# alexj94/future_urban_scene_generation

Measured on NVIDIA B200. Metric: vehicle crops/s novel-view completion (warp+VUNet), higher is better.
Workload: dtype bf16

## Files before the change

future_urban_scene_generation_b200/_lib.py:

```python
import ctypes as C
import os

_HERE = os.path.dirname(os.path.abspath(__file__))
LIB_PATH = os.path.join(_HERE, "libfusg.so")

POLY_COORD_MAX = 1 << 20
ERRORS = {-1: "FUSG_ERR_ARG", -2: "FUSG_ERR_UNSUPPORTED", -3: "FUSG_ERR_CUDA", -4: "FUSG_ERR_WORKSPACE"}


class FusgError(RuntimeError):
    pass


def _load():
    if not os.path.exists(LIB_PATH):
        raise FusgError(
            f"{LIB_PATH} not found: build it with `python -c 'import __graft_entry__ as g; g.build()'` "
            "(nvcc, sm_100a).  There is no CPU fallback for this path.")
    lib = C.CDLL(LIB_PATH)
    vp, sz, i = C.c_void_p, C.c_size_t, C.c_int
    sigs = {
        "fusg_version": ([], i),
        "fusg_last_error": ([], C.c_char_p),
        "fusg_kernel_launches": ([], i),
        "fusg_warp_workspace_bytes": ([i], sz),
        "fusg_warp_workspace_bytes_hw": ([i, i, i], sz),
        "fusg_warp_fused": ([vp] * 11 + [vp, sz, i, i, i, vp], i),
        "fusg_warp_fused_traj": ([vp] * 12 + [vp, sz, i, i, i, vp], i),
        "fusg_warp_fused_idx": ([vp, vp, i] + [vp] * 11 + [vp, sz, i, i, i, vp], i),
        "fusg_warp_window_workspace_bytes": ([i, i, i], sz),
        "fusg_warp_fused_window": ([vp, vp, i] + [vp] * 9 + [i] + [vp] * 4 + [vp, sz, i, i, i, vp], i),
        "fusg_step_keypoints": ([vp] * 10 + [i, i, i, vp], i),
        "fusg_visibility": ([vp] * 6 + [i, i, i, vp], i),
        "fusg_get_planes": ([vp] * 3 + [i, i, i, vp], i),
        "fusg_find_homography": ([vp, vp, i, vp, vp, i, vp], i),
        "fusg_warp_perspective": ([vp] * 3 + [i, i, i, vp], i),
        "fusg_conv2d": ([vp, vp], i),
        "fusg_conv2d_select": ([vp], i),
        "fusg_conv2d_last_plan": ([vp], None),
        "fusg_conv2d_set_sm_reserve": ([i], i),
        "fusg_sizeof_conv_desc": ([], sz),
        "fusg_fold_weightnorm": ([vp, vp, vp, i, i, i, i, i, i, vp], i),
        "fusg_fold_weightnorm_paired": ([vp, vp, vp, vp, vp, i, i, i, i, i, i, vp], i),
        "fusg_nchw_to_nhwc": ([vp, vp, i, i, i, i, i, i, i, vp], i),
        "fusg_nhwc_to_nchw": ([vp, vp, i, i, i, i, i, i, vp], i),
        "fusg_to_image": ([vp, vp, i, i, i, vp], i),
        "fusg_to_image_lab": ([vp, vp, vp, vp, i, i, i, vp], i),
        "fusg_elu": ([vp, vp, sz, i, vp], i),
        "fusg_nchw_to_nhwc_reflect": ([vp, vp, i, i, i, i, i, i, i, vp], i),
        "fusg_norm_stats": ([vp, vp, i, i, i, i, i, vp], i),
        "fusg_norm_finalize": ([vp, vp, vp, vp, i, i, i, i, i, C.c_float, vp], i),
        "fusg_norm_apply": ([vp, vp, vp, i, vp, i, i, i, i, i, i, i, i, vp], i),
        "fusg_resize_u8": ([vp] * 6 + [i, i, vp], i),
        "fusg_paste_workspace_bytes": ([i, i, i], sz),
# ... 26 lines not shown
    return _lib


def check(rc, what):
    if rc != 0:
        msg = lib().fusg_last_error().decode() if rc == -3 else ""
        raise FusgError(f"{what} failed: {ERRORS.get(rc, rc)} {msg}")


def conv_last_plan():
    buf = (C.c_int32 * 8)()
    lib().fusg_conv2d_last_plan(buf)
    return dict(zip(("msub", "pair", "halo", "ksplit", "stages", "group", "w_resident", "fast_epi"), list(buf)))


def kernel_launches():
    return lib().fusg_kernel_launches()


def require_cuda():
    import torch
    if not torch.cuda.is_available():
        raise FusgError("no CUDA device: the B200 path has no CPU fallback")
    return torch


def ptr(t):
    if t is None:
        return None
    assert t.is_cuda and t.is_contiguous(), "expected a contiguous CUDA tensor"
# ... 6 lines not shown
```

future_urban_scene_generation_b200/csrc/conv.cu:

```cuda
#include <cuda.h>
#include <cuda_bf16.h>
#include <cuda_fp16.h>
#include <type_traits>
#include <cuda_runtime.h>
#include <cstdint>
#include <cstdio>
#include <cstring>
#include "../../include/fusg.h"
#include "fusg_common.h"

namespace fusg {

__device__ __forceinline__ float elu1(float x) {
    float e;
    asm("ex2.approx.ftz.f32 %0, %1;" : "=f"(e) : "f"(x * 1.4426950408889634f));
    return x > 0.f ? x : e - 1.f;
}

template <typename T> __device__ __forceinline__ float to_f(T v);
template <> __device__ __forceinline__ float to_f<float>(float v) { return v; }
template <> __device__ __forceinline__ float to_f<__nv_bfloat16>(__nv_bfloat16 v) { return __bfloat162float(v); }
template <> __device__ __forceinline__ float to_f<__half>(__half v) { return __half2float(v); }
template <typename T> __device__ __forceinline__ T from_f(float v);
template <> __device__ __forceinline__ float from_f<float>(float v) { return v; }
// ... 163 lines not shown
    }
    if (active) epilogue16<T>(d, d.bias, Ho, Wo, b, y, x, n0, acc);
}

__device__ __forceinline__ uint32_t s_addr(const void *p) { return (uint32_t)__cvta_generic_to_shared(p); }

__device__ __forceinline__ void mbar_init(uint64_t *bar, uint32_t count) {
    asm volatile("mbarrier.init.shared::cta.b64 [%0], %1;" ::"r"(s_addr(bar)), "r"(count));
}
__device__ __forceinline__ void mbar_arrive_expect_tx(uint64_t *bar, uint32_t bytes) {
    asm volatile("mbarrier.arrive.expect_tx.shared::cta.b64 _, [%0], %1;" ::"r"(s_addr(bar)), "r"(bytes) : "memory");
}
__device__ __forceinline__ void mbar_arrive(uint64_t *bar) {
    asm volatile("mbarrier.arrive.shared::cta.b64 _, [%0];" ::"r"(s_addr(bar)) : "memory");
}
constexpr unsigned TC_WAIT_COUNTER_OFF = 312;
__device__ __forceinline__ void mbar_wait(uint64_t *bar, uint32_t parity) {
    uint32_t done = 0;
    while (!done) {
        asm volatile(
            "{\n\t.reg .pred p;\n\t"
            "mbarrier.try_wait.parity.shared::cta.b64 p, [%1], %2, %3;\n\t"
            "selp.u32 %0, 1, 0, p;\n\t}"
            : "=r"(done)
            : "r"(s_addr(bar)), "r"(parity), "r"(0x989680u)
            : "memory");
        if (!done) fusg_wait_failed((s_addr(bar) & ~1023u) + TC_WAIT_COUNTER_OFF);
    }
}
__device__ __forceinline__ void tma_load_4d(void *dst, const CUtensorMap *tm, uint64_t *bar, int c0, int c1, int c2, int c3) {
    asm volatile(
// ... 237 lines not shown
            v.x = __uint_as_float(acc[c]) + s_bias[c];
            v.y = __uint_as_float(acc[cq + c]) + s_bias[cq + c];
            *reinterpret_cast<float2 *>(p + c * plane) = v;
        }
    }
}

constexpr int TC_EPI_WARPS = 8;
constexpr int TC_THREADS = 64 + 32 * TC_EPI_WARPS;
constexpr int TC_STAGING_BYTES = 32768;
constexpr int TC_STAGE_BYTES = TC_STAGING_BYTES / TC_EPI_WARPS;
constexpr int TC_BLOCK_M = 128;
constexpr int TC_HALO_ROWS_MAX = TC_BLOCK_M + 6;
constexpr int TC_HALO_BYTES = ((TC_HALO_ROWS_MAX * 128 + 1023) / 1024) * 1024;
constexpr int TC_MAX_STAGES = 16;
static_assert(TC_WAIT_COUNTER_OFF == (2 * TC_MAX_STAGES + 5) * 8 + 16, "the wait guard's start-time slot must be tmem_slot[4]");

struct alignas(64) ConvTcParams {
    CUtensorMap tmA0, tmA1, tmW;
    fusg_conv_desc d;
    int Ho, Wo;
    int Wt, Ht, Bt;
    int wt_shift, ht_shift;
    int txs, tys;
    int msub;
    int tiles_x, tiles_y, tiles_b;
    int n_tiles, block_n;
    int kc;
    int chunks0, chunks1;
    int num_kblocks;
    int stages;
    int a_bytes, b_bytes;
    int group;
    int w_resident;
    int halo;
    int hks;
    uint32_t halo_skip;
    int pair;
    int epi_smem;
    unsigned long long w_prefetch_bytes;
    int ksplit;
    int kb_local;
    int tmem_cols;
    int fast_epi;
    FastEpi fe;
};

struct TcSmem { size_t b, bias, stage, total; };
__host__ __device__ __forceinline__ TcSmem tc_smem(const ConvTcParams &p) {
    const size_t pipe_a = p.halo ? (size_t)p.stages * 2 * TC_HALO_BYTES : (size_t)p.stages * p.group * p.a_bytes;
    const size_t pipe_b = p.w_resident ? (size_t)p.num_kblocks * p.b_bytes
                                       : (p.halo ? (size_t)p.stages * p.hks * p.b_bytes : (size_t)p.stages * p.group * p.b_bytes);
    TcSmem s;
    s.b = 1024 + pipe_a;
    s.bias = s.b + ((pipe_b + 15) & ~(size_t)15);
    s.stage = s.bias + (size_t)p.d.cout_pad * 4;
    s.total = 1024  + s.b + pipe_b + 16  + (size_t)p.d.cout_pad * 4 + (size_t)p.epi_smem;
    return s;
}

template <int KSTEPS, int MSUB>
__device__ __forceinline__ void mma_role(const ConvTcParams &p, uint8_t *sA, uint8_t *sB, uint64_t *full_bar, uint64_t *empty_bar,
                                         uint64_t *tfull_bar, uint64_t *tempty_bar, uint64_t *w_bar, uint32_t tmem_base, int total_tiles) {
    const uint32_t block_n = (uint32_t)p.block_n;
    const uint32_t idesc = (1u << 4) | (p.fe.f16 ? 0u : ((1u << 7) | (1u << 10))) | ((block_n >> 3) << 17) | ((uint32_t)(TC_BLOCK_M >> 4) << 24);
    const uint32_t kc = KSTEPS * 16;
    const uint64_t desc_hi = ((uint64_t)1 << 16) | ((uint64_t)((kc * 2u * 8u) >> 4) << 32) | ((uint64_t)1 << 46) | ((uint64_t)(KSTEPS == 4 ? 2u : 4u) << 61);
    const uint32_t sub16 = (TC_BLOCK_M * kc * 2u) >> 4;
    const int group = p.group, stages = p.stages, groups = p.kb_local / p.group;
    const uint32_t a_kb16 = (uint32_t)p.a_bytes >> 4, b_kb16 = (uint32_t)p.b_bytes >> 4;
    const uint32_t a_stage16 = a_kb16 * group, b_stage16 = b_kb16 * group;
    const bool resident = p.w_resident != 0;
    const uint32_t sA16 = (s_addr(sA) & 0x3FFFF) >> 4, sB16 = (s_addr(sB) & 0x3FFFF) >> 4;
    const uint32_t acc_cols = (uint32_t)MSUB * block_n;
    int stage = 0;
    uint32_t phase = 0;
// ... 17 lines not shown
#pragma unroll
                        for (int ks = 0; ks < KSTEPS; ++ks) {
                            umma_bf16(d_tmem + (uint32_t)sub * block_n, a_desc + (uint64_t)(sub * sub16 + ks * 2), b_desc + (uint64_t)(ks * 2), idesc,
                                      ks == 0 ? first : 1u);
                        }
                    }
                    a16 += a_kb16;
                    b16 += b_kb16;
                }
                umma_commit(&empty_bar[stage]);
                if (grp == groups - 1) umma_commit(&tfull_bar[acc]);
            }
            __syncwarp();
            if (++stage == stages) { stage = 0; phase ^= 1; }
        }
        acc ^= 1;
        if (acc == 0) acc_phase ^= 1;
    }
}

template <bool PAIR, int KS>
__device__ __forceinline__ void mma_role_halo(const ConvTcParams &p, uint8_t *sA, uint8_t *sB, uint64_t *full_bar, uint64_t *empty_bar,
                                              uint64_t *tfull_bar, uint64_t *tempty_bar, uint64_t *w_bar, uint32_t tmem_base, int total_tiles) {
    const uint32_t block_n = (uint32_t)p.block_n;
    constexpr bool pair = PAIR;
    if (pair && cluster_ctarank() != 0) return;
    const uint32_t idesc = (1u << 4) | (p.fe.f16 ? 0u : ((1u << 7) | (1u << 10))) | ((block_n >> 3) << 17) | ((uint32_t)((pair ? 2 * TC_BLOCK_M : TC_BLOCK_M) >> 4) << 24);
    const uint64_t desc_hi = ((uint64_t)1 << 16) | ((uint64_t)(1024u >> 4) << 32) | ((uint64_t)1 << 46) | ((uint64_t)2u << 61);
    const int stages = p.stages, cpt = p.chunks0 + p.chunks1, nst = KS * cpt;
    const uint32_t skip = p.halo_skip;
    int st_first = 0, st_last = nst - 1;
    while ((skip >> st_first) & 1u) ++st_first;
    while ((skip >> st_last) & 1u) --st_last;
    const uint32_t b_kb16 = (uint32_t)p.b_bytes >> 4;
    const uint32_t a_stage16 = (2u * TC_HALO_BYTES) >> 4, b_stage16 = (uint32_t)KS * b_kb16;
    const bool resident = p.w_resident != 0;
// ... 36 lines not shown
                } else {
#pragma unroll 1
                    for (int kx = 0; kx < KS; ++kx) issue_tap(kx);
                }
                if constexpr (PAIR) {
                    umma_commit_2cta(&empty_bar[stage]);
                    if (st == st_last) umma_commit_2cta(&tfull_bar[acc]);
                } else {
                    umma_commit(&empty_bar[stage]);
                    if (st == st_last) umma_commit(&tfull_bar[acc]);
                }
            }
            __syncwarp();
            if (++stage == stages) { stage = 0; phase ^= 1; }
        }
        acc ^= 1;
        if (acc == 0) acc_phase ^= 1;
    }
}

template <bool PAIR>
__global__ void __launch_bounds__(TC_THREADS, 1) k_conv_tc(const __grid_constant__ ConvTcParams p) {
    extern __shared__ __align__(1024) uint8_t smem_raw[];
    uint8_t *smem = reinterpret_cast<uint8_t *>((reinterpret_cast<uintptr_t>(smem_raw) + 1023) & ~(uintptr_t)1023);
    const TcSmem lay = tc_smem(p);
    uint64_t *bars = reinterpret_cast<uint64_t *>(smem);
    uint8_t *sA = smem + 1024;
    uint8_t *sB = smem + lay.b;
    uint64_t *full_bar = bars, *empty_bar = bars + TC_MAX_STAGES, *tfull_bar = bars + 2 * TC_MAX_STAGES, *tempty_bar = tfull_bar + 2;
    uint64_t *w_bar = tempty_bar + 2;
    uint32_t *tmem_slot = reinterpret_cast<uint32_t *>(w_bar + 1);
    float *s_bias = reinterpret_cast<float *>(smem + lay.bias);
    uint8_t *s_stage = reinterpret_cast<uint8_t *>(s_bias + p.d.cout_pad);
    float *s_recv = reinterpret_cast<float *>(s_stage);

    const int warp = threadIdx.x >> 5, lane = threadIdx.x & 31;
    const fusg_conv_desc &d = p.d;

    if (warp == 0 && lane == 0) {
        tma_prefetch_desc(&p.tmA0);
        if (d.in1) tma_prefetch_desc(&p.tmA1);
        tma_prefetch_desc(&p.tmW);
        for (int s = 0; s < p.stages; ++s) { mbar_init(&full_bar[s], 1); mbar_init(&empty_bar[s], 1); }
        for (int a = 0; a < 2; ++a) { mbar_init(&tfull_bar[a], 1); mbar_init(&tempty_bar[a], PAIR ? 2 * TC_EPI_WARPS : TC_EPI_WARPS); }
        mbar_init(w_bar, 1);
        fusg_wait_guard_start(tmem_slot + 4);
        asm volatile("fence.mbarrier_init.release.cluster;" ::: "memory");
    }
    if (warp == 1) {
        if constexpr (PAIR) tmem_alloc2(tmem_slot, (uint32_t)p.tmem_cols);
        else tmem_alloc(tmem_slot, (uint32_t)p.tmem_cols);
    }
    for (int i = threadIdx.x; i < p.d.cout_pad; i += TC_THREADS) s_bias[i] = p.d.bias[i];
    tc_fence_before();
    __syncthreads();
    if constexpr (PAIR) cluster_sync_all();
    tc_fence_after();
    const uint32_t tmem_base = *tmem_slot;
    if (p.w_prefetch_bytes && threadIdx.x == 32) {
        const unsigned long long total = p.w_prefetch_bytes, per = ((total / gridDim.x) + 15ull) & ~15ull;
        unsigned long long lo = per * blockIdx.x, hi = lo + per < total ? lo + per : total;
        const char *wb = reinterpret_cast<const char *>(d.weight);
        for (; lo < hi; lo += 32768ull) {
            const unsigned n = (unsigned)(hi - lo < 32768ull ? hi - lo : 32768ull) & ~15u;
            if (n) asm volatile("cp.async.bulk.prefetch.L2.global [%0], %1;" ::"l"(wb + lo), "r"(n) : "memory");
        }
    }
    asm volatile("griddepcontrol.wait;" ::: "memory");
    asm volatile("griddepcontrol.launch_dependents;" ::: "memory");
    if (p.ksplit > 1) asm volatile("barrier.cluster.arrive.relaxed.aligned;" ::: "memory");

    const int m_tiles = p.tiles_x * p.tiles_y * p.tiles_b;
    const int total_tiles = m_tiles * p.n_tiles;
    const int pad = d.pad_mode ? d.pad - d.border : d.ksize >> 1;
    const int cpt = p.chunks0 + p.chunks1;
    int split_tile = -1;

    if (warp == 0) {
        {
            const int groups = p.kb_local / p.group;
            const int kb0 = p.ksplit > 1 ? (int)cluster_ctarank() * p.kb_local : 0;
            const uint32_t stage_tx = (uint32_t)(p.group * (p.a_bytes + (p.w_resident ? 0 : p.b_bytes)));
            if (p.w_resident) {
                if (elect_one()) {
                    mbar_arrive_expect_tx(w_bar, (uint32_t)(p.num_kblocks * p.b_bytes));
// ... 67 lines not shown
                            if (cidx < p.chunks0) tma_load_4d(a_dst, &p.tmA0, &full_bar[stage], cidx * p.kc, ixb + kx, iyb + ky, b0);
                            else tma_load_4d(a_dst, &p.tmA1, &full_bar[stage], (cidx - p.chunks0) * p.kc, ixb + kx, iyb + ky, b0);
                            if (!p.w_resident) tma_load_2d(b_dst, &p.tmW, &full_bar[stage], kcol, n0);
                        }
                        b_dst += p.b_bytes;
                        a_dst += p.a_bytes;
                        kcol += p.kc;
                        if (++cidx == cpt) { cidx = 0; if (++kx == d.ksize) { kx = 0; ++ky; } }
                    }
                    __syncwarp();
                    if (++stage == p.stages) { stage = 0; phase ^= 1; }
                }
            }
        }
    } else if (warp == 1) {
        if (p.halo) {
            if constexpr (PAIR) mma_role_halo<true, 3>(p, sA, sB, full_bar, empty_bar, tfull_bar, tempty_bar, w_bar, tmem_base, total_tiles);
            else if (p.hks == 3) mma_role_halo<false, 3>(p, sA, sB, full_bar, empty_bar, tfull_bar, tempty_bar, w_bar, tmem_base, total_tiles);
            else if (p.hks == 5) mma_role_halo<false, 5>(p, sA, sB, full_bar, empty_bar, tfull_bar, tempty_bar, w_bar, tmem_base, total_tiles);
            else mma_role_halo<false, 7>(p, sA, sB, full_bar, empty_bar, tfull_bar, tempty_bar, w_bar, tmem_base, total_tiles);
        }
        else if (p.kc == 64) {
            if (p.msub == 2) mma_role<4, 2>(p, sA, sB, full_bar, empty_bar, tfull_bar, tempty_bar, w_bar, tmem_base, total_tiles);
            else mma_role<4, 1>(p, sA, sB, full_bar, empty_bar, tfull_bar, tempty_bar, w_bar, tmem_base, total_tiles);
        } else {
            if (p.msub == 2) mma_role<2, 2>(p, sA, sB, full_bar, empty_bar, tfull_bar, tempty_bar, w_bar, tmem_base, total_tiles);
            else mma_role<2, 1>(p, sA, sB, full_bar, empty_bar, tfull_bar, tempty_bar, w_bar, tmem_base, total_tiles);
        }
    } else {
        const int q = warp & 3;
        const int part = (warp - 2) >> 2;
        const int row = q * 32 + lane;
        int nparts = TC_EPI_WARPS / 4;
        while (nparts > 1 && p.block_n % (16 * nparts)) nparts >>= 1;
        const bool sub_split = nparts == 1 && p.msub == 2 && p.ksplit == 1;
        const int ncols = sub_split ? p.block_n : (part < nparts ? p.block_n / nparts : 0);
        const int c_begin = sub_split ? 0 : part * ncols;
        int acc = 0;
        uint32_t acc_phase = 0;
        constexpr bool pair = PAIR;
        const int prank = pair ? (int)cluster_ctarank() : 0;
        const uint32_t tempty_lead0 = pair ? dsmem_addr(s_addr(&tempty_bar[0]), 0) : 0u, tempty_lead1 = pair ? dsmem_addr(s_addr(&tempty_bar[1]), 0) : 0u;
        const int e_step = pair ? (int)gridDim.x >> 1 : (int)gridDim.x / p.ksplit, e_count = pair ? total_tiles >> 1 : total_tiles;
        for (int it = pair ? (int)blockIdx.x >> 1 : (int)blockIdx.x / p.ksplit; it < e_count; it += e_step) {
            const int tile = pair ? 2 * it + prank : it;
            const int mt = p.n_tiles == 1 ? tile : tile / p.n_tiles, nt = tile - mt * p.n_tiles;
            const int tx = mt & (p.tiles_x - 1), ty = (mt >> p.txs) & (p.tiles_y - 1), tb = mt >> (p.txs + p.tys);
            if (p.ksplit > 1) {
                mbar_wait(&tfull_bar[0], 0);
                tc_fence_after();
                const int S = p.ksplit, cpc = (p.block_n >> 4) / S;
                const uint32_t me = cluster_ctarank();
                const uint32_t recv = s_addr(s_recv);
                const uint32_t t_base = tmem_base + ((uint32_t)(q * 32) << 16) + (uint32_t)c_begin;
                asm volatile("barrier.cluster.wait.aligned;" ::: "memory");
                for (int c = 0; c < ncols; c += 16) {
                    uint32_t r[16];
                    tmem_ld16(t_base + (uint32_t)c, r);
                    tmem_ld_wait();
                    const int ch = (c_begin + c) >> 4, owner = ch / cpc, jc = ch - owner * cpc;
                    const uint32_t dst = dsmem_addr(recv + (uint32_t)((((int)me * TC_BLOCK_M + row) * cpc + jc) * 64), (uint32_t)owner);
#pragma unroll
                    for (int i = 0; i < 4; ++i)
// ... 28 lines not shown
                            for (int c = 0; c < ncols; c += 64) asm volatile("prefetch.global.L2 [%0];" ::"l"(rp2 + c));
                        }
                    }
                }
                for (int sub = 0; sub < p.msub; ++sub) {
                    const int trow = row + sub * TC_BLOCK_M;
                    const int wt = trow & (p.Wt - 1), ht = (trow >> p.wt_shift) & (p.Ht - 1), bt = trow >> (p.wt_shift + p.ht_shift);
                    const int ox = tx * p.Wt + wt, oy = ty * p.Ht + ht, b = tb * p.Bt + bt;
                    const size_t opix = ((size_t)b * p.Ho + oy) * p.Wo + ox;
                    const bool valid = b < d.B;
                    const __nv_bfloat16 *rp = fe.res + opix * d.cout + n_base;
                    if (fe.res && valid) {
                        for (int c = 0; c < ncols; c += 64) asm volatile("prefetch.global.L2 [%0];" ::"l"(rp + c));
                    }
                    const size_t off0 = fast_out_offset(fe, d.cout, p.Ho, p.Wo, b, oy, ox - lane, n_base + 8 * jr);
                    if (!waited) { mbar_wait(&tfull_bar[acc], acc_phase); tc_fence_after(); waited = true; }
                    const uint32_t t_base = tmem_base + ((uint32_t)(q * 32) << 16) + (uint32_t)((acc * p.msub + sub) * p.block_n + c_begin);
                    uint32_t r[16];
                    tmem_ld16(t_base, r);
                    for (int c = 0; c < ncols; c += 16) {
                        tmem_ld_wait();
                        float v[16];
                        const float4 *b4 = reinterpret_cast<const float4 *>(s_bias + n_base + c);
#pragma unroll
                        for (int i = 0; i < 4; ++i) {
                            const float4 bb = b4[i];
                            v[4 * i] = __uint_as_float(r[4 * i]) + bb.x;
                            v[4 * i + 1] = __uint_as_float(r[4 * i + 1]) + bb.y;
                            v[4 * i + 2] = __uint_as_float(r[4 * i + 2]) + bb.z;
                            v[4 * i + 3] = __uint_as_float(r[4 * i + 3]) + bb.w;
                        }
                        if (c + 16 < ncols) tmem_ld16(t_base + (uint32_t)(c + 16), r);
// ... 7 lines not shown
#pragma unroll
                            for (int i = 0; i < 8; ++i) { v[2 * i] += bf16lo_to_f(w[i]); v[2 * i + 1] += bf16hi_to_f(w[i]); }
                        }
                        if (fe.f16) {
                            sts128(s0, make_uint4(pack_f16x2(v[0], v[1]), pack_f16x2(v[2], v[3]), pack_f16x2(v[4], v[5]), pack_f16x2(v[6], v[7])));
                            sts128(s1, make_uint4(pack_f16x2(v[8], v[9]), pack_f16x2(v[10], v[11]), pack_f16x2(v[12], v[13]), pack_f16x2(v[14], v[15])));
                        } else {
                            sts128(s0, make_uint4(pack_bf16x2(v[0], v[1]), pack_bf16x2(v[2], v[3]), pack_bf16x2(v[4], v[5]), pack_bf16x2(v[6], v[7])));
                            sts128(s1, make_uint4(pack_bf16x2(v[8], v[9]), pack_bf16x2(v[10], v[11]), pack_bf16x2(v[12], v[13]), pack_bf16x2(v[14], v[15])));
                        }
                    }
                    __syncwarp();
                    if (sub == p.msub - 1) {
                        tc_fence_before();
                        if (lane == 0) {
                            if constexpr (PAIR) mbar_arrive_cluster(acc ? tempty_lead1 : tempty_lead0);
                            else mbar_arrive(&tempty_bar[acc]);
                        }
                    }
                    if (valid) {
                        for (int rw = rw0; rw < 32; rw += rw_step) {
                            const uint4 val = lds128(stg + (uint32_t)(((rw << ppr_shift) + (jr ^ ((rw >> rp_shift) & (ppr - 1)))) << 4));
                            const size_t off = off0 + (size_t)((rw >> 1) * fe.stride_a + (rw & 1) * fe.stride_b);
                            if (fe.raw) *reinterpret_cast<uint4 *>(fe.raw + off) = val;
                            if (fe.elu) *reinterpret_cast<uint4 *>(fe.elu + off) = elu_piece(val);
                        }
                    }
                    __syncwarp();
                }
                if (++acc == 2) { acc = 0; acc_phase ^= 1; }
                continue;
            }
            if (p.fast_epi && p.fe.res && ncols > 0) {
                for (int sub = 0; sub < p.msub; ++sub) {
                    if (sub_split && sub != part) continue;
                    const int trow = row + sub * TC_BLOCK_M;
                    const int wt = trow & (p.Wt - 1), ht = (trow >> p.wt_shift) & (p.Ht - 1), bt = trow >> (p.wt_shift + p.ht_shift);
                    const int b = tb * p.Bt + bt;
                    if (b < d.B) {
                        const size_t opix = ((size_t)b * p.Ho + ty * p.Ht + ht) * p.Wo + tx * p.Wt + wt;
                        const __nv_bfloat16 *rp = p.fe.res + opix * d.cout + nt * p.block_n + c_begin;
                        for (int c = 0; c < ncols; c += 64) asm volatile("prefetch.global.L2 [%0];" ::"l"(rp + c));
                    }
                }
            }
            mbar_wait(&tfull_bar[acc], acc_phase);
            tc_fence_after();
            for (int sub = 0; sub < p.msub && ncols > 0; ++sub) {
                if (sub_split && sub != part) continue;
                const int trow = row + sub * TC_BLOCK_M;
                const int wt = trow & (p.Wt - 1), ht = (trow >> p.wt_shift) & (p.Ht - 1), bt = trow >> (p.wt_shift + p.ht_shift);
                const int ox = tx * p.Wt + wt, oy = ty * p.Ht + ht, b = tb * p.Bt + bt;
                const size_t opix = ((size_t)b * p.Ho + oy) * p.Wo + ox;
                const uint32_t t_base = tmem_base + ((uint32_t)(q * 32) << 16) + (uint32_t)((acc * p.msub + sub) * p.block_n + c_begin);
                uint32_t r[16];
                tmem_ld16(t_base, r);
                for (int c = 0; c < ncols; c += 16) {
                    tmem_ld_wait();
                    uint32_t rr[16];
#pragma unroll
                    for (int i = 0; i < 16; ++i) rr[i] = r[i];
                    if (c + 16 < ncols) tmem_ld16(t_base + (uint32_t)(c + 16), r);
                    if (b < d.B) {
                        const int n = nt * p.block_n + c_begin + c;
                        if (p.fast_epi == 3) unpair_chunk(reinterpret_cast<float *>(p.fe.raw), s_bias, d.cout >> 1, p.Ho, p.Wo, b, oy, ox, rr);
                        else if (p.fast_epi) fast_chunk16(p.fe, s_bias, d.cout, p.Ho, p.Wo, opix, b, oy, ox, n, rr);
                        else {
                            float v[16];
#pragma unroll
                            for (int i = 0; i < 16; ++i) v[i] = __uint_as_float(rr[i]);
                            epilogue16<__nv_bfloat16>(d, s_bias, p.Ho, p.Wo, b, oy, ox, n, v);
                        }
                    }
                }
            }
            tc_fence_before();
            __syncwarp();
            if (lane == 0) {
                if constexpr (PAIR) mbar_arrive_cluster(acc ? tempty_lead1 : tempty_lead0);
                else mbar_arrive(&tempty_bar[acc]);
            }
            if (++acc == 2) { acc = 0; acc_phase ^= 1; }
        }
    }
    if (p.ksplit > 1) {
        __syncwarp();
        if (warp < 2) asm volatile("barrier.cluster.wait.aligned;" ::: "memory");
        cluster_sync_all();
        if (warp >= 2 && split_tile >= 0) {
            const int q = warp & 3, part = (warp - 2) >> 2, row = q * 32 + lane;
            const int S = p.ksplit, cpc = (p.block_n >> 4) / S;
            const int crank = (int)cluster_ctarank();
            const int mt = p.n_tiles == 1 ? split_tile : split_tile / p.n_tiles, nt = split_tile - mt * p.n_tiles;
            const int tx = mt & (p.tiles_x - 1), ty = (mt >> p.txs) & (p.tiles_y - 1), tb = mt >> (p.txs + p.tys);
            const int wt = row & (p.Wt - 1), ht = (row >> p.wt_shift) & (p.Ht - 1), bt = row >> (p.wt_shift + p.ht_shift);
            const int ox = tx * p.Wt + wt, oy = ty * p.Ht + ht, b = tb * p.Bt + bt;
            const size_t opix = ((size_t)b * p.Ho + oy) * p.Wo + ox;
            const float4 *recv = reinterpret_cast<const float4 *>(s_recv);
            for (int j = part; j < cpc; j += TC_EPI_WARPS / 4) {
                float v[16];
// ... 185 lines not shown
    if (!is_pow2(Ho) || !is_pow2(Wo)) return false;
    if (d.cout_pad > 128 && d.cout_pad % 128 != 0) return false;
    if (d.pitch0 % 8 != 0 || (d.in1 && d.pitch1 % 8 != 0)) return false;
    return get_encode() != nullptr;
}

static int g_sm_reserve = 0;

extern "C" int fusg_conv2d_set_sm_reserve(int n) {
    const int prev = g_sm_reserve;
    if (n >= 0) g_sm_reserve = n;
    return prev;
}

static thread_local int32_t g_last_plan[8];

extern "C" void fusg_conv2d_last_plan(int32_t *plan8) {
    for (int i = 0; i < 8; ++i) plan8[i] = g_last_plan[i];
}

static int plan_tc(const fusg_conv_desc &d, int Ho, int Wo, int num_sms, ConvTcParams &p, int &grid, size_t &smem) {
    memset(&p, 0, sizeof(p));
    p.d = d;
    p.Ho = Ho; p.Wo = Wo;
    p.block_n = d.cout_pad < 128 ? d.cout_pad : 128;
    p.n_tiles = d.cout_pad / p.block_n;
    const long long rows = (long long)d.B * Ho * Wo;
    p.msub = (rows / 256 * p.n_tiles >= 4LL * num_sms && rows % 256 == 0) ? 2 : 1;
    const int trows = TC_BLOCK_M * p.msub;
    p.Wt = Wo < 128 ? Wo : 128;
    p.Ht = (trows / p.Wt) < Ho ? (trows / p.Wt) : Ho;
    p.Bt = trows / (p.Wt * p.Ht);
    p.tiles_x = Wo / p.Wt; p.tiles_y = Ho / p.Ht; p.tiles_b = (d.B + p.Bt - 1) / p.Bt;
    const int total_tiles = p.tiles_x * p.tiles_y * p.tiles_b * p.n_tiles;
// ... 93 lines not shown
        p.fast_epi = ok ? (want_staged ? 2 : 1) : 0;
        if (!ok && p.ksplit == 1 && d.noise == nullptr && d.residual == nullptr && d.dtype == FUSG_DTYPE_BF16 && d.cout <= 16 && d.cout % 2 == 0 && p.block_n == 16) {
            int nouts = 0;
            const fusg_conv_out *only = nullptr;
            for (int sidx = 0; sidx < FUSG_CONV_MAX_OUTS; ++sidx)
                if (d.outs[sidx].ptr) { ++nouts; only = &d.outs[sidx]; }
            if (nouts == 1 && only->layout == 1 && only->mode == FUSG_OUT_UNPAIR && only->source == 0 && only->elu == 0 &&
                (reinterpret_cast<uintptr_t>(only->ptr) & 7) == 0) {
                memset(&fe, 0, sizeof(fe));
                fe.raw = reinterpret_cast<__nv_bfloat16 *>(only->ptr);
                p.fast_epi = 3;
            }
        }
        p.fe = fe;
    }
    const unsigned long long wbytes = (unsigned long long)d.cout_pad * taps * (d.c0 + d.c1) * 2ull;
    p.w_prefetch_bytes = (total_tiles * p.ksplit <= 64 && wbytes >= 65536ull && (reinterpret_cast<uintptr_t>(d.weight) & 15) == 0) ? wbytes : 0ull;
    const int usable = num_sms - g_sm_reserve > 8 ? num_sms - g_sm_reserve : num_sms;
    grid = p.ksplit > 1 ? total_tiles * p.ksplit  : (total_tiles < usable ? total_tiles : usable);
    if (p.pair) grid &= ~1;
    smem = tc_smem(p).total;
    return FUSG_OK;
}

static int launch_tc(const fusg_conv_desc &d, int Ho, int Wo, cudaStream_t st) {
    ConvTcParams p;
    int grid;
    size_t smem;
    const int rc = plan_tc(d, Ho, Wo, fusg_num_sms(), p, grid, smem);
    if (rc != FUSG_OK) return rc;
// ... 12 lines not shown
    };
    if (!encodeA(&p.tmA0, d.in0, d.cphys0 ? d.cphys0 : d.c0, d.pitch0)) return FUSG_ERR_UNSUPPORTED;
    if (d.in1 && !encodeA(&p.tmA1, d.in1, d.cphys1 ? d.cphys1 : d.c1, d.pitch1)) return FUSG_ERR_UNSUPPORTED;
    {
        const int ktot = d.ksize * d.ksize * (d.c0 + d.c1);
        cuuint64_t dims[2] = {(cuuint64_t)ktot, (cuuint64_t)d.cout_pad};
        cuuint64_t strides[1] = {(cuuint64_t)ktot * 2};
        cuuint32_t box[2] = {(cuuint32_t)p.kc, (cuuint32_t)(p.pair ? p.block_n / 2 : p.block_n)};
        cuuint32_t estr[2] = {1, 1};
        if (enc(&p.tmW, d.dtype == FUSG_DTYPE_F16 ? CU_TENSOR_MAP_DATA_TYPE_FLOAT16 : CU_TENSOR_MAP_DATA_TYPE_BFLOAT16, 2, const_cast<void *>(d.weight), dims, strides, box, estr,
                CU_TENSOR_MAP_INTERLEAVE_NONE, sw, CU_TENSOR_MAP_L2_PROMOTION_L2_256B, CU_TENSOR_MAP_FLOAT_OOB_FILL_NONE) != CUDA_SUCCESS)
            return FUSG_ERR_UNSUPPORTED;
    }
    if (fusg_once_per_device(0, 0, [] {
            cudaError_t e = cudaFuncSetAttribute(k_conv_tc<false>, cudaFuncAttributeMaxDynamicSharedMemorySize, 227 * 1024);
            return e != cudaSuccess ? e : cudaFuncSetAttribute(k_conv_tc<true>, cudaFuncAttributeMaxDynamicSharedMemorySize, 227 * 1024);
        }) != cudaSuccess)
        return fusg_check_launch();
    g_last_plan[0] = p.msub; g_last_plan[1] = p.pair; g_last_plan[2] = p.halo; g_last_plan[3] = p.ksplit;
    g_last_plan[4] = p.stages; g_last_plan[5] = p.group; g_last_plan[6] = p.w_resident; g_last_plan[7] = p.fast_epi;
    cudaLaunchConfig_t cfg;
    memset(&cfg, 0, sizeof(cfg));
    cfg.gridDim = dim3((unsigned)grid, 1, 1);
    cfg.blockDim = dim3(TC_THREADS, 1, 1);
    cfg.dynamicSmemBytes = smem;
    cfg.stream = st;
    cudaLaunchAttribute attr[2];
    attr[0].id = cudaLaunchAttributeProgrammaticStreamSerialization;
    attr[0].val.programmaticStreamSerializationAllowed = 1;
    int na = 1;
    if (p.ksplit > 1 || p.pair) {
        attr[na].id = cudaLaunchAttributeClusterDimension;
        attr[na].val.clusterDim.x = p.pair ? 2u : (unsigned)p.ksplit;
        attr[na].val.clusterDim.y = 1;
        attr[na].val.clusterDim.z = 1;
        ++na;
    }
    cfg.attrs = attr;
    cfg.numAttrs = (unsigned)na;
    if ((p.pair ? cudaLaunchKernelEx(&cfg, k_conv_tc<true>, p) : cudaLaunchKernelEx(&cfg, k_conv_tc<false>, p)) != cudaSuccess) return fusg_check_launch();
    fusg_count_launch(1);
    return fusg_check_launch();
}

extern "C" size_t fusg_sizeof_conv_desc(void) { return sizeof(fusg_conv_desc); }

constexpr int SC_THREADS = 256;
constexpr int SC_CIN = 8;
constexpr int SC_PIX = 4;

__global__ void __launch_bounds__(SC_THREADS, 2) k_conv1x1_smallcin(const __nv_bfloat16 *__restrict__ in, int pitch_in, const __nv_bfloat16 *__restrict__ w,
                                                                    int cin_pad, const float *__restrict__ bias, __nv_bfloat16 *__restrict__ raw,
                                                                    __nv_bfloat16 *__restrict__ elu, int cout, long long npix) {
    const int chunks = cout >> 3;
    const int chunk = threadIdx.x % chunks, pl = threadIdx.x / chunks, ppc = SC_THREADS / chunks;
// ... 187 lines not shown
```

include/fusg.h:

```cpp
#ifndef FUSG_H_
#define FUSG_H_

#include <stddef.h>
#include <stdint.h>

#ifdef __cplusplus
extern "C" {
#endif

#define FUSG_OK 0
#define FUSG_ERR_ARG (-1)
#define FUSG_ERR_UNSUPPORTED (-2)
#define FUSG_ERR_CUDA (-3)
#define FUSG_ERR_WORKSPACE (-4)

int fusg_version(void);
const char *fusg_last_error(void);
int fusg_kernel_launches(void);


size_t fusg_warp_workspace_bytes(int B);
size_t fusg_warp_workspace_bytes_hw(int B, int H, int W);

int fusg_warp_fused(const uint8_t *src, const int32_t *src_kp, const int32_t *dst_kp,
// ... 73 lines not shown
    const float *noise;
    fusg_conv_out outs[FUSG_CONV_MAX_OUTS];
    int32_t dtype;
    int32_t impl;
    uint64_t zero_kblocks;
    int32_t pad_mode;
    int32_t pad, border;
    int32_t cphys0, cphys1;
    int32_t cin_real;
} fusg_conv_desc;

int fusg_conv2d(const fusg_conv_desc *desc, void *stream);
size_t fusg_sizeof_conv_desc(void);
int fusg_conv2d_select(const fusg_conv_desc *desc);
void fusg_conv2d_last_plan(int32_t *plan8_host);
int fusg_conv2d_set_sm_reserve(int n);

int fusg_fold_weightnorm(const float *v, const float *g, void *w_out, int cout, int cin, int ksize,
                         int cout_pad, int cin_pad, int dtype, void *stream);

int fusg_fold_weightnorm_paired(const float *v, const float *g, const float *bias, void *w_out, float *bias_out,
                                int cout, int cin0, int cin1, int ksize, int cout_pad, int dtype, void *stream);

int fusg_nchw_to_nhwc(const float *in, void *out, int B, int C, int H, int W, int cpad, int elu, int dtype, void *stream);
int fusg_nhwc_to_nchw(const void *in, float *out, int B, int C, int H, int W, int pitch, int dtype, void *stream);
int fusg_to_image(const float *in, uint8_t *out, int B, int H, int W, void *stream);
int fusg_to_image_lab(const float *in, uint8_t *out, const uint16_t *lab_to_yf, const uint8_t *inv_gamma, int B, int H, int W, void *stream);
int fusg_resize_u8(const uint8_t *src, const long long *src_off, const int32_t *src_hw, uint8_t *dst, const long long *dst_off,
                   const int32_t *dst_hw, int B, int max_dst_pixels, void *stream);
size_t fusg_paste_workspace_bytes(int F, int Hf, int Wf);
// ... 52 lines not shown
```

Before: 7907.

## Add grouped-epilogue conv kernel with 3-4 TMEM accumulators and per-group epilogue warps

Adds a variant of the tcgen05 conv kernel for single-CTA, non-split, bf16, small-N layers. It runs 3 or 4 epilogue warpgroups, each owning its own TMEM accumulator and tile stream, so the MMA warp can run several tiles ahead of the epilogue drain. This targets layers where the epilogue, not the MMA, is the bottleneck. In exchange it uses more threads, more TMEM columns and more epilogue smem, and recomputes the pipeline stage count, which can reduce stages.

```diff
diff --git a/future_urban_scene_generation_b200/_lib.py b/future_urban_scene_generation_b200/_lib.py
--- a/future_urban_scene_generation_b200/_lib.py
+++ b/future_urban_scene_generation_b200/_lib.py
@@ -38,6 +38,7 @@
         "fusg_conv2d": ([vp, vp], i),
         "fusg_conv2d_select": ([vp], i),
         "fusg_conv2d_last_plan": ([vp], None),
+        "fusg_conv2d_last_epi_groups": ([], i),
         "fusg_conv2d_set_sm_reserve": ([i], i),
         "fusg_sizeof_conv_desc": ([], sz),
         "fusg_fold_weightnorm": ([vp, vp, vp, i, i, i, i, i, i, vp], i),
@@ -94,6 +95,10 @@
     return dict(zip(("msub", "pair", "halo", "ksplit", "stages", "group", "w_resident", "fast_epi"), list(buf)))
 
 
+def conv_last_epi_groups():
+    return lib().fusg_conv2d_last_epi_groups()
+
+
 def kernel_launches():
     return lib().fusg_kernel_launches()
 
diff --git a/future_urban_scene_generation_b200/csrc/conv.cu b/future_urban_scene_generation_b200/csrc/conv.cu
--- a/future_urban_scene_generation_b200/csrc/conv.cu
+++ b/future_urban_scene_generation_b200/csrc/conv.cu
@@ -201,7 +201,7 @@
 __device__ __forceinline__ void mbar_arrive(uint64_t *bar) {
     asm volatile("mbarrier.arrive.shared::cta.b64 _, [%0];" ::"r"(s_addr(bar)) : "memory");
 }
-constexpr unsigned TC_WAIT_COUNTER_OFF = 312;
+constexpr unsigned TC_WAIT_COUNTER_OFF = 344;
 __device__ __forceinline__ void mbar_wait(uint64_t *bar, uint32_t parity) {
     uint32_t done = 0;
     while (!done) {
@@ -469,7 +469,9 @@
 constexpr int TC_HALO_ROWS_MAX = TC_BLOCK_M + 6;
 constexpr int TC_HALO_BYTES = ((TC_HALO_ROWS_MAX * 128 + 1023) / 1024) * 1024;
 constexpr int TC_MAX_STAGES = 16;
-static_assert(TC_WAIT_COUNTER_OFF == (2 * TC_MAX_STAGES + 5) * 8 + 16, "the wait guard's start-time slot must be tmem_slot[4]");
+constexpr int TC_MAX_ACC = 4;
+static_assert(TC_WAIT_COUNTER_OFF == (2 * TC_MAX_STAGES + 2 * TC_MAX_ACC + 1) * 8 + 16, "the wait guard's start-time slot must be tmem_slot[4]");
+static_assert(TC_WAIT_COUNTER_OFF + 8 <= 1024, "the barrier block must fit its 1024 bytes");
 
 struct alignas(64) ConvTcParams {
     CUtensorMap tmA0, tmA1, tmW;
@@ -498,6 +500,7 @@
     int kb_local;
     int tmem_cols;
     int fast_epi;
+    int epi_groups;
     FastEpi fe;
 };
 
@@ -514,7 +517,7 @@
     return s;
 }
 
-template <int KSTEPS, int MSUB>
+template <int KSTEPS, int MSUB, int NACC>
 __device__ __forceinline__ void mma_role(const ConvTcParams &p, uint8_t *sA, uint8_t *sB, uint64_t *full_bar, uint64_t *empty_bar,
                                          uint64_t *tfull_bar, uint64_t *tempty_bar, uint64_t *w_bar, uint32_t tmem_base, int total_tiles) {
     const uint32_t block_n = (uint32_t)p.block_n;
@@ -562,12 +565,11 @@
             __syncwarp();
             if (++stage == stages) { stage = 0; phase ^= 1; }
         }
-        acc ^= 1;
-        if (acc == 0) acc_phase ^= 1;
-    }
-}
-
-template <bool PAIR, int KS>
+        if (++acc == NACC) { acc = 0; acc_phase ^= 1; }
+    }
+}
+
+template <bool PAIR, int KS, int NACC>
 __device__ __forceinline__ void mma_role_halo(const ConvTcParams &p, uint8_t *sA, uint8_t *sB, uint64_t *full_bar, uint64_t *empty_bar,
                                               uint64_t *tfull_bar, uint64_t *tempty_bar, uint64_t *w_bar, uint32_t tmem_base, int total_tiles) {
     const uint32_t block_n = (uint32_t)p.block_n;
@@ -634,21 +636,25 @@
             __syncwarp();
             if (++stage == stages) { stage = 0; phase ^= 1; }
         }
-        acc ^= 1;
-        if (acc == 0) acc_phase ^= 1;
-    }
-}
-
-template <bool PAIR>
-__global__ void __launch_bounds__(TC_THREADS, 1) k_conv_tc(const __grid_constant__ ConvTcParams p) {
+        if (++acc == NACC) { acc = 0; acc_phase ^= 1; }
+    }
+}
+
+template <int EPI_GROUPS> __host__ __device__ constexpr int tc_threads() { return EPI_GROUPS > 1 ? 64 + 128 * EPI_GROUPS : TC_THREADS; }
+
+template <bool PAIR, int EPI_GROUPS = 1>
+__global__ void __launch_bounds__(tc_threads<EPI_GROUPS>(), 1) k_conv_tc(const __grid_constant__ ConvTcParams p) {
+    static_assert(EPI_GROUPS == 1 || (!PAIR && EPI_GROUPS <= TC_MAX_ACC), "grouped epilogue: single CTAs, one accumulator per group");
+    constexpr bool grouped = EPI_GROUPS > 1;
+    constexpr int NACC = grouped ? EPI_GROUPS : 2;
     extern __shared__ __align__(1024) uint8_t smem_raw[];
     uint8_t *smem = reinterpret_cast<uint8_t *>((reinterpret_cast<uintptr_t>(smem_raw) + 1023) & ~(uintptr_t)1023);
     const TcSmem lay = tc_smem(p);
     uint64_t *bars = reinterpret_cast<uint64_t *>(smem);
     uint8_t *sA = smem + 1024;
     uint8_t *sB = smem + lay.b;
-    uint64_t *full_bar = bars, *empty_bar = bars + TC_MAX_STAGES, *tfull_bar = bars + 2 * TC_MAX_STAGES, *tempty_bar = tfull_bar + 2;
-    uint64_t *w_bar = tempty_bar + 2;
+    uint64_t *full_bar = bars, *empty_bar = bars + TC_MAX_STAGES, *tfull_bar = bars + 2 * TC_MAX_STAGES, *tempty_bar = tfull_bar + TC_MAX_ACC;
+    uint64_t *w_bar = tempty_bar + TC_MAX_ACC;
     uint32_t *tmem_slot = reinterpret_cast<uint32_t *>(w_bar + 1);
     float *s_bias = reinterpret_cast<float *>(smem + lay.bias);
     uint8_t *s_stage = reinterpret_cast<uint8_t *>(s_bias + p.d.cout_pad);
@@ -662,7 +668,7 @@
         if (d.in1) tma_prefetch_desc(&p.tmA1);
         tma_prefetch_desc(&p.tmW);
         for (int s = 0; s < p.stages; ++s) { mbar_init(&full_bar[s], 1); mbar_init(&empty_bar[s], 1); }
-        for (int a = 0; a < 2; ++a) { mbar_init(&tfull_bar[a], 1); mbar_init(&tempty_bar[a], PAIR ? 2 * TC_EPI_WARPS : TC_EPI_WARPS); }
+        for (int a = 0; a < NACC; ++a) { mbar_init(&tfull_bar[a], 1); mbar_init(&tempty_bar[a], PAIR ? 2 * TC_EPI_WARPS : (grouped ? 4 : TC_EPI_WARPS)); }
         mbar_init(w_bar, 1);
         fusg_wait_guard_start(tmem_slot + 4);
         asm volatile("fence.mbarrier_init.release.cluster;" ::: "memory");
@@ -671,7 +677,7 @@
         if constexpr (PAIR) tmem_alloc2(tmem_slot, (uint32_t)p.tmem_cols);
         else tmem_alloc(tmem_slot, (uint32_t)p.tmem_cols);
     }
-    for (int i = threadIdx.x; i < p.d.cout_pad; i += TC_THREADS) s_bias[i] = p.d.bias[i];
+    for (int i = threadIdx.x; i < p.d.cout_pad; i += tc_threads<EPI_GROUPS>()) s_bias[i] = p.d.bias[i];
     tc_fence_before();
     __syncthreads();
     if constexpr (PAIR) cluster_sync_all();
@@ -688,7 +694,7 @@
     }
     asm volatile("griddepcontrol.wait;" ::: "memory");
     asm volatile("griddepcontrol.launch_dependents;" ::: "memory");
-    if (p.ksplit > 1) asm volatile("barrier.cluster.arrive.relaxed.aligned;" ::: "memory");
+    if (!grouped && p.ksplit > 1) asm volatile("barrier.cluster.arrive.relaxed.aligned;" ::: "memory");
 
     const int m_tiles = p.tiles_x * p.tiles_y * p.tiles_b;
     const int total_tiles = m_tiles * p.n_tiles;
@@ -786,39 +792,55 @@
             }
         }
     } else if (warp == 1) {
-        if (p.halo) {
-            if constexpr (PAIR) mma_role_halo<true, 3>(p, sA, sB, full_bar, empty_bar, tfull_bar, tempty_bar, w_bar, tmem_base, total_tiles);
-            else if (p.hks == 3) mma_role_halo<false, 3>(p, sA, sB, full_bar, empty_bar, tfull_bar, tempty_bar, w_bar, tmem_base, total_tiles);
-            else if (p.hks == 5) mma_role_halo<false, 5>(p, sA, sB, full_bar, empty_bar, tfull_bar, tempty_bar, w_bar, tmem_base, total_tiles);
-            else mma_role_halo<false, 7>(p, sA, sB, full_bar, empty_bar, tfull_bar, tempty_bar, w_bar, tmem_base, total_tiles);
+        if constexpr (grouped) {
+            if (p.halo) mma_role_halo<false, 3, NACC>(p, sA, sB, full_bar, empty_bar, tfull_bar, tempty_bar, w_bar, tmem_base, total_tiles);
+            else if (p.msub == 2) mma_role<4, 2, NACC>(p, sA, sB, full_bar, empty_bar, tfull_bar, tempty_bar, w_bar, tmem_base, total_tiles);
+            else mma_role<4, 1, NACC>(p, sA, sB, full_bar, empty_bar, tfull_bar, tempty_bar, w_bar, tmem_base, total_tiles);
+        } else if (p.halo) {
+            if constexpr (PAIR) mma_role_halo<true, 3, NACC>(p, sA, sB, full_bar, empty_bar, tfull_bar, tempty_bar, w_bar, tmem_base, total_tiles);
+            else if (p.hks == 3) mma_role_halo<false, 3, NACC>(p, sA, sB, full_bar, empty_bar, tfull_bar, tempty_bar, w_bar, tmem_base, total_tiles);
+            else if (p.hks == 5) mma_role_halo<false, 5, NACC>(p, sA, sB, full_bar, empty_bar, tfull_bar, tempty_bar, w_bar, tmem_base, total_tiles);
+            else mma_role_halo<false, 7, NACC>(p, sA, sB, full_bar, empty_bar, tfull_bar, tempty_bar, w_bar, tmem_base, total_tiles);
         }
         else if (p.kc == 64) {
-            if (p.msub == 2) mma_role<4, 2>(p, sA, sB, full_bar, empty_bar, tfull_bar, tempty_bar, w_bar, tmem_base, total_tiles);
-            else mma_role<4, 1>(p, sA, sB, full_bar, empty_bar, tfull_bar, tempty_bar, w_bar, tmem_base, total_tiles);
+            if (p.msub == 2) mma_role<4, 2, NACC>(p, sA, sB, full_bar, empty_bar, tfull_bar, tempty_bar, w_bar, tmem_base, total_tiles);
+            else mma_role<4, 1, NACC>(p, sA, sB, full_bar, empty_bar, tfull_bar, tempty_bar, w_bar, tmem_base, total_tiles);
         } else {
-            if (p.msub == 2) mma_role<2, 2>(p, sA, sB, full_bar, empty_bar, tfull_bar, tempty_bar, w_bar, tmem_base, total_tiles);
-            else mma_role<2, 1>(p, sA, sB, full_bar, empty_bar, tfull_bar, tempty_bar, w_bar, tmem_base, total_tiles);
+            if (p.msub == 2) mma_role<2, 2, NACC>(p, sA, sB, full_bar, empty_bar, tfull_bar, tempty_bar, w_bar, tmem_base, total_tiles);
+            else mma_role<2, 1, NACC>(p, sA, sB, full_bar, empty_bar, tfull_bar, tempty_bar, w_bar, tmem_base, total_tiles);
         }
     } else {
         const int q = warp & 3;
-        const int part = (warp - 2) >> 2;
+        const int part = grouped ? 0 : (warp - 2) >> 2;
+        const int egrp = grouped ? (warp - 2) >> 2 : 0;
         const int row = q * 32 + lane;
-        int nparts = TC_EPI_WARPS / 4;
+        int nparts = grouped ? 1 : TC_EPI_WARPS / 4;
         while (nparts > 1 && p.block_n % (16 * nparts)) nparts >>= 1;
-        const bool sub_split = nparts == 1 && p.msub == 2 && p.ksplit == 1;
+        const bool sub_split = !grouped && nparts == 1 && p.msub == 2 && p.ksplit == 1;
         const int ncols = sub_split ? p.block_n : (part < nparts ? p.block_n / nparts : 0);
         const int c_begin = sub_split ? 0 : part * ncols;
         int acc = 0;
         uint32_t acc_phase = 0;
+        auto cur_acc = [&]() -> int {
+            if constexpr (grouped) {
+                uint32_t t;
+                asm volatile("mov.u32 %0, %%tid.x;" : "=r"(t));
+                return (int)(t - 64u) >> 7;
+            } else {
+                return acc;
+            }
+        };
         constexpr bool pair = PAIR;
         const int prank = pair ? (int)cluster_ctarank() : 0;
         const uint32_t tempty_lead0 = pair ? dsmem_addr(s_addr(&tempty_bar[0]), 0) : 0u, tempty_lead1 = pair ? dsmem_addr(s_addr(&tempty_bar[1]), 0) : 0u;
-        const int e_step = pair ? (int)gridDim.x >> 1 : (int)gridDim.x / p.ksplit, e_count = pair ? total_tiles >> 1 : total_tiles;
-        for (int it = pair ? (int)blockIdx.x >> 1 : (int)blockIdx.x / p.ksplit; it < e_count; it += e_step) {
+        const int e_step = pair ? (int)gridDim.x >> 1 : (grouped ? (int)gridDim.x * EPI_GROUPS : (int)gridDim.x / p.ksplit);
+        const int e_count = pair ? total_tiles >> 1 : total_tiles;
+        const int e_first = pair ? (int)blockIdx.x >> 1 : (grouped ? (int)blockIdx.x + egrp * (int)gridDim.x : (int)blockIdx.x / p.ksplit);
+        for (int it = e_first; it < e_count; it += e_step) {
             const int tile = pair ? 2 * it + prank : it;
             const int mt = p.n_tiles == 1 ? tile : tile / p.n_tiles, nt = tile - mt * p.n_tiles;
             const int tx = mt & (p.tiles_x - 1), ty = (mt >> p.txs) & (p.tiles_y - 1), tb = mt >> (p.txs + p.tys);
-            if (p.ksplit > 1) {
+            if (!grouped && p.ksplit > 1) {
                 mbar_wait(&tfull_bar[0], 0);
                 tc_fence_after();
                 const int S = p.ksplit, cpc = (p.block_n >> 4) / S;
@@ -877,8 +899,8 @@
                         for (int c = 0; c < ncols; c += 64) asm volatile("prefetch.global.L2 [%0];" ::"l"(rp + c));
                     }
                     const size_t off0 = fast_out_offset(fe, d.cout, p.Ho, p.Wo, b, oy, ox - lane, n_base + 8 * jr);
-                    if (!waited) { mbar_wait(&tfull_bar[acc], acc_phase); tc_fence_after(); waited = true; }
-                    const uint32_t t_base = tmem_base + ((uint32_t)(q * 32) << 16) + (uint32_t)((acc * p.msub + sub) * p.block_n + c_begin);
+                    if (!waited) { mbar_wait(&tfull_bar[cur_acc()], acc_phase); tc_fence_after(); waited = true; }
+                    const uint32_t t_base = tmem_base + ((uint32_t)(q * 32) << 16) + (uint32_t)((cur_acc() * p.msub + sub) * p.block_n + c_begin);
                     uint32_t r[16];
                     tmem_ld16(t_base, r);
                     for (int c = 0; c < ncols; c += 16) {
@@ -916,8 +938,8 @@
                     if (sub == p.msub - 1) {
                         tc_fence_before();
                         if (lane == 0) {
-                            if constexpr (PAIR) mbar_arrive_cluster(acc ? tempty_lead1 : tempty_lead0);
-                            else mbar_arrive(&tempty_bar[acc]);
+                            if constexpr (PAIR) mbar_arrive_cluster(cur_acc() ? tempty_lead1 : tempty_lead0);
+                            else mbar_arrive(&tempty_bar[cur_acc()]);
                         }
                     }
                     if (valid) {
@@ -930,7 +952,8 @@
                     }
                     __syncwarp();
                 }
-                if (++acc == 2) { acc = 0; acc_phase ^= 1; }
+                if (grouped) acc_phase ^= 1;
+                else if (++acc == 2) { acc = 0; acc_phase ^= 1; }
                 continue;
             }
             if (p.fast_epi && p.fe.res && ncols > 0) {
@@ -946,7 +969,7 @@
                     }
                 }
             }
-            mbar_wait(&tfull_bar[acc], acc_phase);
+            mbar_wait(&tfull_bar[cur_acc()], acc_phase);
             tc_fence_after();
             for (int sub = 0; sub < p.msub && ncols > 0; ++sub) {
                 if (sub_split && sub != part) continue;
@@ -954,7 +977,7 @@
                 const int wt = trow & (p.Wt - 1), ht = (trow >> p.wt_shift) & (p.Ht - 1), bt = trow >> (p.wt_shift + p.ht_shift);
                 const int ox = tx * p.Wt + wt, oy = ty * p.Ht + ht, b = tb * p.Bt + bt;
                 const size_t opix = ((size_t)b * p.Ho + oy) * p.Wo + ox;
-                const uint32_t t_base = tmem_base + ((uint32_t)(q * 32) << 16) + (uint32_t)((acc * p.msub + sub) * p.block_n + c_begin);
+                const uint32_t t_base = tmem_base + ((uint32_t)(q * 32) << 16) + (uint32_t)((cur_acc() * p.msub + sub) * p.block_n + c_begin);
                 uint32_t r[16];
                 tmem_ld16(t_base, r);
                 for (int c = 0; c < ncols; c += 16) {
@@ -965,7 +988,8 @@
                     if (c + 16 < ncols) tmem_ld16(t_base + (uint32_t)(c + 16), r);
                     if (b < d.B) {
                         const int n = nt * p.block_n + c_begin + c;
-                        if (p.fast_epi == 3) unpair_chunk(reinterpret_cast<float *>(p.fe.raw), s_bias, d.cout >> 1, p.Ho, p.Wo, b, oy, ox, rr);
+                        if constexpr (grouped) fast_chunk16(p.fe, s_bias, d.cout, p.Ho, p.Wo, opix, b, oy, ox, n, rr);
+                        else if (p.fast_epi == 3) unpair_chunk(reinterpret_cast<float *>(p.fe.raw), s_bias, d.cout >> 1, p.Ho, p.Wo, b, oy, ox, rr);
                         else if (p.fast_epi) fast_chunk16(p.fe, s_bias, d.cout, p.Ho, p.Wo, opix, b, oy, ox, n, rr);
                         else {
                             float v[16];
@@ -979,13 +1003,14 @@
             tc_fence_before();
             __syncwarp();
             if (lane == 0) {
-                if constexpr (PAIR) mbar_arrive_cluster(acc ? tempty_lead1 : tempty_lead0);
-                else mbar_arrive(&tempty_bar[acc]);
-            }
-            if (++acc == 2) { acc = 0; acc_phase ^= 1; }
-        }
-    }
-    if (p.ksplit > 1) {
+                if constexpr (PAIR) mbar_arrive_cluster(cur_acc() ? tempty_lead1 : tempty_lead0);
+                else mbar_arrive(&tempty_bar[cur_acc()]);
+            }
+            if (grouped) acc_phase ^= 1;
+            else if (++acc == 2) { acc = 0; acc_phase ^= 1; }
+        }
+    }
+    if (!grouped && p.ksplit > 1) {
         __syncwarp();
         if (warp < 2) asm volatile("barrier.cluster.wait.aligned;" ::: "memory");
         cluster_sync_all();
@@ -1201,10 +1226,13 @@
 }
 
 static thread_local int32_t g_last_plan[8];
+static thread_local int32_t g_last_epi_groups = 0;
 
 extern "C" void fusg_conv2d_last_plan(int32_t *plan8) {
     for (int i = 0; i < 8; ++i) plan8[i] = g_last_plan[i];
 }
+
+extern "C" int fusg_conv2d_last_epi_groups(void) { return g_last_epi_groups; }
 
 static int plan_tc(const fusg_conv_desc &d, int Ho, int Wo, int num_sms, ConvTcParams &p, int &grid, size_t &smem) {
     memset(&p, 0, sizeof(p));
@@ -1328,6 +1356,22 @@
         }
         p.fe = fe;
     }
+    p.epi_groups = 1;
+    if (p.ksplit == 1 && !p.pair && (p.fast_epi == 1 || p.fast_epi == 2) && d.noise == nullptr && d.dtype == FUSG_DTYPE_BF16 &&
+        d.pad_mode == 0 && d.stride == 1 && p.kc == 64 && is_pow2(p.block_n) && p.block_n <= 64 && (long long)Ho * Wo >= 128 * 64) {
+        const int G = (d.ksize == 1 || (p.halo && p.w_resident)) ? 4 : 3;
+        ConvTcParams g = p;
+        g.epi_groups = G;
+        g.epi_smem = p.fast_epi == 2 ? G * 4 * TC_STAGE_BYTES : 0;
+        const int budget = 224 * 1024 - g.epi_smem - (g.w_resident ? g.num_kblocks * g.b_bytes : 0);
+        const int stage_bytes = g.halo ? 2 * TC_HALO_BYTES + (g.w_resident ? 0 : d.ksize * g.b_bytes)
+                                       : g.group * (g.a_bytes + (g.w_resident ? 0 : g.b_bytes));
+        g.stages = budget / stage_bytes < TC_MAX_STAGES ? budget / stage_bytes : TC_MAX_STAGES;
+        int cols = 32;
+        while (cols < G * g.msub * g.block_n) cols <<= 1;
+        g.tmem_cols = cols;
+        if (cols <= 512 && g.stages >= 2 && tc_smem(g).total <= 227 * 1024) p = g;
+    }
     const unsigned long long wbytes = (unsigned long long)d.cout_pad * taps * (d.c0 + d.c1) * 2ull;
     p.w_prefetch_bytes = (total_tiles * p.ksplit <= 64 && wbytes >= 65536ull && (reinterpret_cast<uintptr_t>(d.weight) & 15) == 0) ? wbytes : 0ull;
     const int usable = num_sms - g_sm_reserve > 8 ? num_sms - g_sm_reserve : num_sms;
@@ -1370,15 +1414,18 @@
     }
     if (fusg_once_per_device(0, 0, [] {
             cudaError_t e = cudaFuncSetAttribute(k_conv_tc<false>, cudaFuncAttributeMaxDynamicSharedMemorySize, 227 * 1024);
+            if (e == cudaSuccess) e = cudaFuncSetAttribute(k_conv_tc<false, 3>, cudaFuncAttributeMaxDynamicSharedMemorySize, 227 * 1024);
+            if (e == cudaSuccess) e = cudaFuncSetAttribute(k_conv_tc<false, 4>, cudaFuncAttributeMaxDynamicSharedMemorySize, 227 * 1024);
             return e != cudaSuccess ? e : cudaFuncSetAttribute(k_conv_tc<true>, cudaFuncAttributeMaxDynamicSharedMemorySize, 227 * 1024);
         }) != cudaSuccess)
         return fusg_check_launch();
     g_last_plan[0] = p.msub; g_last_plan[1] = p.pair; g_last_plan[2] = p.halo; g_last_plan[3] = p.ksplit;
     g_last_plan[4] = p.stages; g_last_plan[5] = p.group; g_last_plan[6] = p.w_resident; g_last_plan[7] = p.fast_epi;
+    g_last_epi_groups = p.epi_groups;
     cudaLaunchConfig_t cfg;
     memset(&cfg, 0, sizeof(cfg));
     cfg.gridDim = dim3((unsigned)grid, 1, 1);
-    cfg.blockDim = dim3(TC_THREADS, 1, 1);
+    cfg.blockDim = dim3(p.epi_groups == 4 ? tc_threads<4>() : (p.epi_groups == 3 ? tc_threads<3>() : TC_THREADS), 1, 1);
     cfg.dynamicSmemBytes = smem;
     cfg.stream = st;
     cudaLaunchAttribute attr[2];
@@ -1394,7 +1441,10 @@
     }
     cfg.attrs = attr;
     cfg.numAttrs = (unsigned)na;
-    if ((p.pair ? cudaLaunchKernelEx(&cfg, k_conv_tc<true>, p) : cudaLaunchKernelEx(&cfg, k_conv_tc<false>, p)) != cudaSuccess) return fusg_check_launch();
+    const cudaError_t le = p.pair ? cudaLaunchKernelEx(&cfg, k_conv_tc<true>, p)
+                                  : p.epi_groups == 4 ? cudaLaunchKernelEx(&cfg, k_conv_tc<false, 4>, p)
+                                  : p.epi_groups == 3 ? cudaLaunchKernelEx(&cfg, k_conv_tc<false, 3>, p) : cudaLaunchKernelEx(&cfg, k_conv_tc<false>, p);
+    if (le != cudaSuccess) return fusg_check_launch();
     fusg_count_launch(1);
     return fusg_check_launch();
 }
diff --git a/include/fusg.h b/include/fusg.h
--- a/include/fusg.h
+++ b/include/fusg.h
@@ -111,6 +111,7 @@
 size_t fusg_sizeof_conv_desc(void);
 int fusg_conv2d_select(const fusg_conv_desc *desc);
 void fusg_conv2d_last_plan(int32_t *plan8_host);
+int fusg_conv2d_last_epi_groups(void);
 int fusg_conv2d_set_sm_reserve(int n);
 
 int fusg_fold_weightnorm(const float *v, const float *g, void *w_out, int cout, int cin, int ksize,
```

Result: faster. 8100 (median of 6 runs) (+2.5%).
